# LuisaGroup/LuisaRender

Measured on AMD Instinct MI355X. Metric: Msamples/s (+ fraction of HBM roofline) at fixed SPP, 1/2/4/8 GPU, higher is better.
Workload: dtype f32; 1 GPU; Contemporary Bathroom-class (procedural stand-in, ~600k tris), 1024x1024, 1024spp, depth 16; integrator=MegaPath, sampler=Independent (seed 19980810), spp=1024, parallelism=single GPU, collective=none (single GPU), scheduler=path pool, two contexts per lane (megapool_kernel.h)

## Files before the change

__graft_entry__.py:

```python
import os
import subprocess
import sys

ROOT = os.path.dirname(os.path.abspath(__file__))
if ROOT not in sys.path:
    sys.path.insert(0, ROOT)


def build() -> None:
    jobs = f"-j{min(os.cpu_count() or 4, 16)}"
    subprocess.check_call(["make", "-C", ROOT, jobs, "host", "oracle", "hip", "cli", "ieee", "shallow", "noearly", "nopair", "noride"])
    if os.path.isdir("/root/reference/src"):
        subprocess.check_call(["make", "-C", ROOT, jobs, "ref"])
    import luisarender_amd
    from luisarender_amd import _ffi
    _ffi.host_lib()
    assert os.path.exists(os.path.join(ROOT, "luisarender_amd", "lib", "liblrhip.so"))


def smoke() -> None:
    import numpy as np
    from luisarender_amd import Scene
    from oracle.check import Oracle
    from luisarender_amd.render import MegaPathRenderer
    from luisarender_amd.scenes import cornell_box

    scene = Scene.from_string(cornell_box(resolution=64, spp=8))
    renderer = MegaPathRenderer(0)
    renderer.upload(scene)
    renderer.render(0, 8, counters=True, sync=True)
    gpu = renderer.download(converted=False)
    cpu, counters = Oracle(scene).render(0, 8)
    rel = float(np.abs(gpu[..., :3] - cpu[..., :3]).sum() / np.abs(cpu[..., :3]).sum())
    gc = renderer.counters()
    assert np.array_equal(gpu[..., 3], cpu[..., 3]), "sample counts differ"
    assert abs(gc["closest_rays"] - counters["closest_rays"]) <= 2, (gc, counters)
    assert rel < 1e-4, f"relative L1 vs oracle {rel}"
    print(f"smoke ok: rel L1 vs oracle = {rel:.3e}, {renderer.last_render_ms():.3f} ms")


if __name__ == "__main__":
    build()
    if len(sys.argv) > 1 and sys.argv[1] == "smoke":
        smoke()
```

luisarender_amd/csrc/hip/megapool_kernel.h:

```cpp
#pragma once
#include "dev_wavefront.h"

namespace lrd {

#ifndef LR_MIN_WAVES
#define LR_MIN_WAVES 4
#endif
#ifndef LR_POOL_SHADE_LANES
#define LR_POOL_SHADE_LANES 56
#endif
#ifndef LR_POOL_IDLE_LANES
#define LR_POOL_IDLE_LANES 16
#endif
#ifndef LR_POOL_TURNOVER_LANES
#define LR_POOL_TURNOVER_LANES 12
#endif
#ifndef LR_POOL_PARK_ON_STACK
#define LR_POOL_PARK_ON_STACK 1
#endif
#ifndef LR_POOL_FUSED_FETCH
#define LR_POOL_FUSED_FETCH 1
#endif
#ifndef LR_POOL_FUSED_ALPHA
#define LR_POOL_FUSED_ALPHA 0
#endif
#ifndef LR_POOL_EARLY_FETCH
#define LR_POOL_EARLY_FETCH 1
#endif
#ifndef LR_POOL_LEAF_NODE_PAIR
#define LR_POOL_LEAF_NODE_PAIR 1
#endif
#ifndef LR_POOL_EARLY_TAIL_PRIO
#define LR_POOL_EARLY_TAIL_PRIO 3
#endif
#ifndef LR_POOL_STATE_LEAN
#define LR_POOL_STATE_LEAN 1
#endif
#ifndef LR_POOL_RAY_INIT
#define LR_POOL_RAY_INIT if (!mine)
#endif
#ifndef LR_POOL_SHADOW_RIDE
#define LR_POOL_SHADOW_RIDE 1
#endif
constexpr uint32_t kPoolSlots = 128u;

template<bool GENERIC>
constexpr uint32_t pool_quads() { return GENERIC ? 5u : 4u; }
constexpr uint32_t kPoolRecordQuadsMax = pool_quads<true>() + 1u;
constexpr uint32_t kPoolPending = 1u << 22u;

enum : uint32_t {
    kCtxShadow = 1u, kCtxClosest = 2u,
    kCtxHadShadow = 4u, kCtxHadClosest = 8u,
    kCtxDone = 16u,
    kCtxOccluded = 32u,
    kCtxSide = 64u,
    kCtxOpen = 128u,
};
struct PathCtx {
    f3 so, sd;
    float s_tmax;
    f3 no, nd;
    float n_tmin, n_tmax;
    uint32_t tri;
    float u, v;
    uint32_t flags;
};
LR_D void ctx_start(PathCtx &c, TravState &tr) {
    tr.o = c.no, tr.d = c.nd, tr.t_min = c.n_tmin, tr.t_max = c.n_tmax;
    tr.phase = kPhaseClosest;
    if ((c.flags & kCtxShadow) != 0u) {
        asm volatile("");
        tr.o = c.so, tr.d = c.sd, tr.t_min = 0.f, tr.t_max = c.s_tmax;
        tr.phase = kPhaseShadow;
        c.flags &= ~kCtxShadow;
    } else {
        asm volatile("");
        c.flags &= ~kCtxClosest;
    }
    tr.cur = 0u, tr.sp = 0u;
    tr.hit.tri = kInvalid, tr.hit.u = 0.f, tr.hit.v = 0.f;
    tr.occluded = false;
}

LR_D void swap_words(float &x, float &y) { asm volatile("v_swap_b32 %0, %1" : "+v"(x), "+v"(y)); }
LR_D void swap_words(uint32_t &x, uint32_t &y) { asm volatile("v_swap_b32 %0, %1" : "+v"(x), "+v"(y)); }
LR_D void ctx_swap(PathCtx &a, PathCtx &b) {
    swap_words(a.so.x, b.so.x), swap_words(a.so.y, b.so.y), swap_words(a.so.z, b.so.z), swap_words(a.s_tmax, b.s_tmax);
    swap_words(a.sd.x, b.sd.x), swap_words(a.sd.y, b.sd.y), swap_words(a.sd.z, b.sd.z);
    swap_words(a.no.x, b.no.x), swap_words(a.no.y, b.no.y), swap_words(a.no.z, b.no.z), swap_words(a.n_tmin, b.n_tmin);
    swap_words(a.nd.x, b.nd.x), swap_words(a.nd.y, b.nd.y), swap_words(a.nd.z, b.nd.z), swap_words(a.n_tmax, b.n_tmax);
    swap_words(a.tri, b.tri), swap_words(a.u, b.u), swap_words(a.v, b.v), swap_words(a.flags, b.flags);
}

#ifndef LR_POOL_TURNOVER_MOVES
#define LR_POOL_TURNOVER_MOVES 1
#endif
LR_D void ctx_turnover(PathCtx &a, PathCtx &b) {
    if (LR_POOL_TURNOVER_MOVES == 0) { ctx_swap(a, b); return; }
    a.so = b.so, a.sd = b.sd, a.s_tmax = b.s_tmax, a.n_tmin = b.n_tmin, a.n_tmax = b.n_tmax;
    b.tri = a.tri, b.u = a.u, b.v = a.v;
    swap_words(a.no.x, b.no.x), swap_words(a.no.y, b.no.y), swap_words(a.no.z, b.no.z);
    swap_words(a.nd.x, b.nd.x), swap_words(a.nd.y, b.nd.y), swap_words(a.nd.z, b.nd.z);
    swap_words(a.flags, b.flags);
}

LR_D uint32_t lane_rank(unsigned long long mask) {
    return __builtin_amdgcn_mbcnt_hi(static_cast<uint32_t>(mask >> 32u), __builtin_amdgcn_mbcnt_lo(static_cast<uint32_t>(mask), 0u));
}

constexpr uint32_t kCtxRays = kCtxShadow | kCtxClosest;
LR_D bool ctx_shadeable(uint32_t flags, bool samples_left) {
#ifdef LR_POOL_SINGLE
    if ((flags & kCtxSide) != 0u) { samples_left = false; }
#endif
    return (flags & kCtxDone) != 0u || (samples_left && (flags & kCtxOpen) == 0u);
}
LR_D bool pool_shade_due(uint32_t phase, uint32_t cur_flags, uint32_t oth_flags, bool samples_left) {
    const auto idle = phase == kPhaseIdle;
    const auto s = lr_ballot(ctx_shadeable(oth_flags, samples_left) || (idle && ctx_shadeable(cur_flags, samples_left)));
    if (s == 0ull) { return false; }
    const auto idle_mask = lr_ballot(idle);
    return static_cast<uint32_t>(__popcll(s)) >= static_cast<uint32_t>(LR_POOL_SHADE_LANES) ||
           static_cast<uint32_t>(__popcll(s & idle_mask)) >= static_cast<uint32_t>(LR_POOL_IDLE_LANES) || idle_mask == ~0ull;
}

template<bool COUNT, bool ALPHA>
LR_D bool pool_trace(const DScene &scene, const TraversalStack &stack, TravState &tr, PathCtx &cur, PathCtx &oth, bool samples_left, TraceStats &stats) {
    const auto tl = TravLane::make(scene, stack);
    auto inv = safe_inverse(tr.d);
    auto spb = tl.spb_of(tr.sp);
    if (tr.phase == kPhaseIdle) { tr.cur = kCurIdle; }
    auto for_alpha = false;
    constexpr bool FUSED = LR_POOL_FUSED_FETCH != 0 && (!ALPHA || LR_POOL_FUSED_ALPHA != 0);
    constexpr int EARLY = FUSED ? LR_POOL_EARLY_FETCH : 0;
    constexpr bool PAIR = FUSED && LR_POOL_LEAF_NODE_PAIR != 0;
#ifdef LR_STALL_PROBE
    if (COUNT) { probe_start(stats); }
#endif
    LeafRequest rq;
    [[maybe_unused]] auto asked = tr.cur;
// ... 25 lines not shown
            const auto any_inner = PAIR || lr_any(static_cast<int>(tr.cur) >= 0), deep = lr_any(spb > tl.s_deep);
            trav_consume<COUNT, ALPHA, PAIR>(stack, tl, tr, spb, inv, rq, any_inner, deep, stats);
            trav_requests<COUNT, true, PAIR>(stack, tl, tr, spb, rq, EARLY == 1, stats);
            if (LR_POOL_EARLY_TAIL_PRIO == 0) { prio_tests(); }
            if (COUNT) { asked = tr.cur; }
        } else {
            trav_iteration<COUNT, ALPHA, FUSED, PAIR>(stack, tl, tr, spb, inv, stats);
        }
#ifdef LR_TRACE_PROBE
        const auto probe_t1 = __builtin_readcyclecounter();
        const auto probe_t2 = probe_t1;
#endif
        if (ALPHA && alpha_tests_due(tr.phase, tr.cur)) { for_alpha = true; break; }
        const auto ended = tr.cur == kInvalid;
        const auto n_ended = static_cast<uint32_t>(__popcll(lr_ballot(ended)));
#ifdef LR_TRACE_PROBE
        if (COUNT && (threadIdx.x & 63u) == 0u) {
            stats.nodes_empty += static_cast<uint32_t>(probe_t1 - probe_t0);
            stats.steps_starved += static_cast<uint32_t>(__builtin_readcyclecounter() - probe_t2);
        }
#endif
        if (n_ended == 0u) { continue; }
        if (n_ended < static_cast<uint32_t>(LR_POOL_TURNOVER_LANES) && lr_any(tr.cur < kCurParked)) { continue; }
        if (ended) {
            if (tr.phase == kPhaseShadow) {
                if (tr.occluded) { cur.flags |= kCtxOccluded; }
            } else {
                cur.tri = tr.hit.tri, cur.u = tr.hit.u, cur.v = tr.hit.v;
            }
            tr.phase = kPhaseIdle, tr.cur = kCurIdle;
            if ((cur.flags & kCtxRays) == 0u) {
                cur.flags |= kCtxDone;
                if ((oth.flags & kCtxRays) != 0u) { ctx_turnover(cur, oth); }
            }
            if ((cur.flags & kCtxRays) != 0u) {
                ctx_start(cur, tr);
                inv = safe_inverse(tr.d);
                spb = tl.lds_base;
            }
        }
        if (!lr_any(ended && tr.cur == kCurIdle)) { continue; }
        if (lr_ballot(tr.cur != kCurIdle) == 0ull) { break; }
        if (pool_shade_due(tr.phase, cur.flags, oth.flags, samples_left)) { break; }
    }
    if (EARLY != 0) { trav_fetch_wait(); }
    LR_MARK(kProbeTail, tr.cur);
    prio_shade();
    tr.sp = tl.sp_of(spb);
    return for_alpha;
}

#ifndef LR_PADDED_DRAWS_OUT_OF_LINE
#define LR_PADDED_DRAWS_OUT_OF_LINE 1
#endif
struct PaddedDraws {
    float a, b, c, d;
};
[[maybe_unused]] static __device__ __noinline__ PaddedDraws padded_draws(const DScene *scene, uint32_t sample_index, uint32_t pixel, uint32_t dimension, bool four) {
    PathSampler<true> sampler{};
    uint32_t words[kWfSamplerWordsMax] = {sample_index, 0u, dimension, pixel};
    sampler.restore(*scene, words);
    PaddedDraws r;
    r.a = sampler.next_1d();
    const auto u = sampler.next_2d();
    r.b = u.x, r.c = u.y;
    r.d = four ? sampler.next_1d() : 0.f;
    return r;
}

#ifndef LR_LIGHT_OUT_OF_LINE
#if defined(LR_VARIANT) && ((LR_VARIANT) & 16) && !((LR_VARIANT) & (96 | 256))
#define LR_LIGHT_OUT_OF_LINE 1
#else
#define LR_LIGHT_OUT_OF_LINE 0
#endif
#endif
template<bool ENV>
[[maybe_unused]] static __device__ __noinline__ LightPick sample_one_light_call(const DScene *scene, f3 p, f3 ng, f3 ns, uint32_t offset_bits, float u0, float u1, float u2) {
    SurfacePoint it{};
    it.p = p, it.ng = ng, it.shading.n = ns, it.offset_bits = offset_bits;
    return sample_one_light<ENV>(*scene, it, u0, f2{u1, u2});
}

#define LR_POOL_FILM_ADD(L, PIXEL, OF_ITEM, TILE_PIXEL)                                                                                          \
    do {                                                                                                                                         \
        const auto rgb = (L) * scene.shutter_weight;                                                                                             \
        if (CONT || (OF_ITEM) != item) {                                \
            wf_film_accumulate(scene, args.film, (PIXEL), rgb, scene.film_clamp);                                                                \
        } else if (!(any_nan(rgb) || any_inf(rgb))) {   \
            const auto threshold = scene.film_clamp * fmaxf(1.f, 1.f);                                                                           \
            const auto strength = fmaxf(fmaxf(fmaxf(fabsf(rgb.x), fabsf(rgb.y)), fabsf(rgb.z)), 0.f);                                            \
            const auto c = rgb * (threshold / fmaxf(strength, threshold));                                                                       \
            const auto px_sums = film_tile + (TILE_PIXEL) * 3u;                                                                                  \
            if (c.x != 0.f) { atomicAdd(px_sums + 0, radiance_to_fixed(c.x, scene.wf.accum_scale)); }                                            \
            if (c.y != 0.f) { atomicAdd(px_sums + 1, radiance_to_fixed(c.y, scene.wf.accum_scale)); }                                            \
            if (c.z != 0.f) { atomicAdd(px_sums + 2, radiance_to_fixed(c.z, scene.wf.accum_scale)); }                                            \
        } else {                                                                        \
            atomicAdd(&args.film[(PIXEL)].w, -1.f);                                                                                              \
        }                                                                                                                                        \
    } while (false)

template<uint32_t F>
__global__ __launch_bounds__(kBlockThreads, LR_MIN_WAVES) void megapool_kernel(DScenePtr scene_ptr, RenderArgs args) {
    const DScene &scene = *(const DScene *)scene_ptr;
    constexpr bool COUNT = (F & kFeatCount) != 0u, PCG = (F & kFeatGeneric) != 0u, ENV = (F & kFeatEnv) != 0u,
                   ALPHA = (F & kFeatAlpha) != 0u, DISNEY = (F & kFeatDisney) != 0u, WF = (F & kFeatWf) != 0u, CONT = (F & kFeatCont) != 0u;
    static_assert((F & kFeatPool) != 0u, "a pool variant");
    static_assert(kPoolParkedWords == 5u, "the shading block parks five words on top of a lane's stack (below): lrhip_upload_scene bounds the BVH depth with this constant");
    static_assert((F & (kFeatMix | kFeatLayered | kFeatAux | kFeatVpt | kFeatNest)) == 0u, "the pool scheduler exists for the lean kernels (closures inline)");
    static_assert(!WF || !DISNEY, "a wavefront variant is a lean kernel: the heavy closures live in heavy_kernel.h");
    static_assert(!CONT || WF, "the continuation pass exists in wavefront mode only");
    constexpr uint32_t SAMPLER_WORDS = PathSampler<PCG>::kSavedWords;
#ifdef LR_ONLY_SAMPLER
    constexpr bool PADDED = PCG && (LR_ONLY_SAMPLER) == LR_SAMPLER_PADDED_SOBOL;
#else
    constexpr bool PADDED = false;
#endif
    static_assert(PADDED == ((F & kFeatPadded) != 0u) || (F & kFeatPadded) == 0u, "a kFeatPadded kernel: generic sampler, LR_ONLY_SAMPLER = PaddedSobol");
    constexpr uint32_t QUADS = PADDED ? 4u : pool_quads<PCG>();
    constexpr bool RIDE = LR_POOL_SHADOW_RIDE != 0 && !WF;
    constexpr uint32_t RECORD = QUADS + (RIDE ? 1u : 0u);
    static_assert(RECORD <= kPoolRecordQuadsMax, "ensure_pool sizes the records");
    __shared__ uint32_t s_stack[kStackLds * kBlockThreads];
    __shared__ float4 s_stage[kWavesPerBlock * kStageWave];
#if LR_POOL_PARK_ON_STACK == 0
    __shared__ uint32_t s_park[5u * kBlockThreads];
    static_assert(kStackLds + 5u <= 16u, "the parking area is carved out of the round 1-3 stack: compile such pool variants with LR_STACK_LDS <= 11");
#endif
    __shared__ unsigned long long s_film[CONT ? 1u : kWavesPerBlock * 192u];
#ifdef LR_STALL_PROBE
    __shared__ uint32_t s_probe[kWavesPerBlock * kProbeWords];
    if ((threadIdx.x & 63u) < kProbeWords) { s_probe[(threadIdx.x >> 6u) * kProbeWords + (threadIdx.x & 63u)] = 0u; }
    const auto probe_wave = (F & kFeatCount) != 0u && (blockIdx.x % 9u) == 0u && __builtin_amdgcn_readfirstlane(threadIdx.x >> 6u) == ((blockIdx.x / 9u) & 3u);
#endif
    const auto tid = threadIdx.x;
    const auto lane = tid & 63u;
    const auto gtid = blockIdx.x * kBlockThreads + tid;
    const auto wave_in_block = __builtin_amdgcn_readfirstlane(tid >> 6u);
    TraversalStack stack{s_stack + tid, args.spill + gtid, args.total_threads, s_stage + wave_in_block * kStageWave};
    const auto film_tile = s_film + (CONT ? 0u : wave_in_block * 192u);
    const auto state_of = [&](uint32_t side, uint32_t quad) { return args.pool + static_cast<size_t>(side * RECORD + quad) * args.total_threads + gtid; };
    const auto state_load = [&](uint32_t side, uint32_t quad) { return *state_of(side, quad); };
    const auto state_store = [&](uint32_t side, uint32_t quad, float4 v) { *state_of(side, quad) = v; };
    DCounters local{};
    const auto t_wave = COUNT ? __builtin_readcyclecounter() : 0ull;

    const auto cont_total = CONT ? min(scene.wf.counts[kWfCountCont], scene.wf.capacity) : 0u;
    const auto cont_waves = gridDim.x * kWavesPerBlock;
    const auto item_records = CONT ? min(kWfItemRecords, max(64u, ((cont_total + cont_waves - 1u) / cont_waves + 63u) & ~63u)) : 1u;
    const auto item_count = CONT ? (cont_total + item_records - 1u) / item_records : args.item_count;
    const auto cont_queue = wf_cont_queue(scene);

    auto item = kInvalid;
    auto items_left = true;
    auto q_next = 0u, q_total = 0u;
    auto s_begin = 0u, s_count = 0u, tx = 0u, ty = 0u;
    if (!CONT) { film_tile[lane * 3u] = 0ull, film_tile[lane * 3u + 1u] = 0ull, film_tile[lane * 3u + 2u] = 0ull; }
    TravState tr{};
    tr.phase = kPhaseIdle;
    PathCtx cur{}, oth{};
    cur.flags = 0u, oth.flags = kCtxSide;

    auto flush_tile = [&]() {
        if (CONT || item == kInvalid) { return; }
        __builtin_amdgcn_fence(__ATOMIC_ACQ_REL, "wavefront");
        __builtin_amdgcn_wave_barrier();
        const auto a0 = film_tile[lane * 3u], a1 = film_tile[lane * 3u + 1u], a2 = film_tile[lane * 3u + 2u];
        film_tile[lane * 3u] = 0ull, film_tile[lane * 3u + 1u] = 0ull, film_tile[lane * 3u + 2u] = 0ull;
        const auto wx = tx * 8u + (lane & 7u), wy = ty * 8u + (lane >> 3u);
        if (wx < scene.camera.width && wy < scene.camera.height) {
            const auto index = wy * scene.camera.width + wx;
            const auto acc = scene.wf.accum + static_cast<size_t>(index) * 3u;
            if (a0 != 0ull) { atomicAdd(acc + 0, a0); }
            if (a1 != 0ull) { atomicAdd(acc + 1, a1); }
            if (a2 != 0ull) { atomicAdd(acc + 2, a2); }
            if (s_count != 0u) { atomicAdd(&args.film[index].w, static_cast<float>(s_count)); }
        }
        __builtin_amdgcn_fence(__ATOMIC_ACQ_REL, "wavefront");
        __builtin_amdgcn_wave_barrier();
    };

    auto take_item = [&]() {
        flush_tile();
        item = next_item(CONT ? scene.wf.counts + kWfWorkCont : args.work_counter, item_count, lane);
        q_next = 0u, q_total = 0u, s_count = 0u;
        if (item == kInvalid) {
            items_left = false;
            return;
        }
        if (CONT) {
            q_total = min(item_records, cont_total - item * item_records);
        } else {
            const auto range = item_range(args, item);
            const auto tile = args.tile_begin + range.tile_index * args.tile_stride;
            ty = tile / args.tiles_x, tx = (tile - ty * args.tiles_x + ty) % args.tiles_x;
            s_begin = range.s_begin, s_count = range.s_end > range.s_begin ? range.s_end - range.s_begin : 0u;
            q_total = s_count * 64u;
        }
    };

    for (;;) {
        for (;;) {
            const auto samples_left = items_left || q_next < q_total;
            if (!pool_shade_due(tr.phase, cur.flags, oth.flags, samples_left)) { break; }
            const auto t_shade = COUNT ? __builtin_readcyclecounter() : 0ull;
            if (ALPHA) { tr.pend_t = 0.f, tr.pend_u = 0.f, tr.pend_v = 0.f; }
            if (tr.phase == kPhaseIdle && !ctx_shadeable(oth.flags, samples_left)) { ctx_swap(cur, oth); }
#ifdef LR_POOL_SINGLE
            const auto mine = (oth.flags & kCtxDone) != 0u || ((oth.flags & kCtxOpen) == 0u && (oth.flags & kCtxSide) == 0u);
#else
            const auto mine = (oth.flags & kCtxDone) != 0u || (oth.flags & kCtxOpen) == 0u;
#endif
            {
                const auto stage = stack.stage;
                stage[lane] = make_float4(cur.so.x, cur.so.y, cur.so.z, cur.s_tmax);
                stage[64u + lane] = make_float4(cur.sd.x, cur.sd.y, cur.sd.z, cur.n_tmin);
                stage[128u + lane] = make_float4(cur.no.x, cur.no.y, cur.no.z, cur.n_tmax);
                const auto keep_word = (tr.phase & 7u) | (tr.occluded ? 8u : 0u) | (tr.sp << 5u) | (cur.flags << 12u) | (oth.flags << 20u);
                stage[192u + lane] = make_float4(cur.nd.x, cur.nd.y, cur.nd.z, __uint_as_float(keep_word));
#if LR_POOL_PARK_ON_STACK
                stack.push(tr.sp + 0u, tr.phase != kPhaseIdle ? tr.hit.tri : cur.tri);
                stack.push(tr.sp + 1u, __float_as_uint(tr.phase != kPhaseIdle ? tr.hit.u : cur.u));
                stack.push(tr.sp + 2u, __float_as_uint(tr.phase != kPhaseIdle ? tr.hit.v : cur.v));
                stack.push(tr.sp + 3u, __float_as_uint(tr.t_max));
                stack.push(tr.sp + 4u, tr.cur);
#else
                const auto park = s_park + tid;
                park[0u * kBlockThreads] = tr.phase != kPhaseIdle ? tr.hit.tri : cur.tri;
                park[1u * kBlockThreads] = __float_as_uint(tr.phase != kPhaseIdle ? tr.hit.u : cur.u);
                park[2u * kBlockThreads] = __float_as_uint(tr.phase != kPhaseIdle ? tr.hit.v : cur.v);
                park[3u * kBlockThreads] = __float_as_uint(tr.t_max);
                park[4u * kBlockThreads] = tr.cur;
#endif
                asm volatile("" ::: "memory");
            }
            PathSampler<PCG> sampler{};
            Ray ray{}, shadow{};
            LR_POOL_RAY_INIT {
                shadow.o = oth.so, shadow.d = oth.sd, shadow.t_min = 0.f, shadow.t_max = oth.s_tmax;
                ray.o = oth.no, ray.d = oth.nd, ray.t_min = oth.n_tmin, ray.t_max = oth.n_tmax;
            }
            f3 beta = mk3(0.f), Li = mk3(0.f), nee = mk3(0.f);
            auto pdf_bsdf = 1e16f;
            auto dp = 0u, pixel_index = 0u, path_item = kInvalid;
            const auto side = (oth.flags & kCtxSide) != 0u ? 1u : 0u;
            auto path_open = (oth.flags & kCtxDone) != 0u;
            const auto traced_shadow = path_open && (oth.flags & kCtxHadShadow) != 0u, traced_closest = path_open && (oth.flags & kCtxHadClosest) != 0u;
            const auto occluded = (oth.flags & kCtxOccluded) != 0u;
            const auto ro = oth.no, rd = oth.nd;
            const auto hit_tri = oth.tri;
            const auto hit_u = oth.u, hit_v = oth.v;
            constexpr bool LEAN_STATE = LR_POOL_STATE_LEAN != 0;
            auto word0 = 0u;
            const auto load_ids = [&]() {
                const auto q3 = state_load(side, 3u);
                pixel_index = __float_as_uint(q3.x), path_item = __float_as_uint(q3.y);
            };
            const auto sampler_take = [&](uint32_t stage) {
                if (PADDED) {
                    const auto q3 = state_load(side, 3u);
                    const auto depth = dp & 0xffffu;
                    const auto first_rr = scene.rr_depth == 0u ? 0u : scene.rr_depth - 1u;
                    const auto dimension = (scene.camera.kind == LR_CAMERA_THIN_LENS ? 4u : 2u) + 6u * depth + (depth > first_rr ? depth - first_rr : 0u) + 3u * stage;
                    uint32_t words[kWfSamplerWordsMax] = {__float_as_uint(q3.z), 0u, dimension, __float_as_uint(q3.w)};
                    sampler.restore(scene, words);
                    return;
                }
                const auto q3 = state_load(side, 3u);
                uint32_t words[kWfSamplerWordsMax] = {word0, __float_as_uint(q3.z), __float_as_uint(q3.w), __float_as_uint(state_load(side, QUADS - 1u).x)};
                sampler.restore(scene, words);
            };
            const auto sampler_leave = [&]() {
                if (PADDED) { return; }
                uint32_t words[kWfSamplerWordsMax] = {0u, 0u, 0u, 0u};
                sampler.save(words);
                word0 = words[0];
                state_store(side, 2u, make_float4(Li.x, Li.y, Li.z, __uint_as_float(words[0])));
                const auto q3 = state_load(side, 3u);
                state_store(side, 3u, make_float4(q3.x, q3.y, __uint_as_float(words[1]), __uint_as_float(words[2])));
                state_store(side, QUADS - 1u, make_float4(__uint_as_float(words[3]), 0.f, 0.f, 0.f));
            };
            auto sampler_left = false;
            if (path_open) {
                const auto q0 = state_load(side, 0u), q1 = state_load(side, 1u), q2 = state_load(side, 2u);
                nee = mk3(q0.x, q0.y, q0.z), pdf_bsdf = q0.w;
                beta = mk3(q1.x, q1.y, q1.z);
                const auto packed = __float_as_uint(q1.w);
                dp = packed & (RIDE ? 0x7fffffu : 0x3fffffu);
                Li = mk3(q2.x, q2.y, q2.z);
                word0 = __float_as_uint(q2.w);
                if (!LEAN_STATE) { load_ids(); }
                if (!PCG) {
                    uint32_t words[kWfSamplerWordsMax] = {word0, 0u, 0u, 0u};
                    sampler.restore(scene, words);
                }
            }
            auto want_shadow = false, want_closest = false;
            unsigned long long t_closure_sum = 0ull;
#ifdef LR_STALL_PROBE
            uint32_t t_lobe = 0u, t_eval = 0u, t_sample = 0u, t_hit = 0u, t_light = 0u;
            const auto probe_clock = []() { return static_cast<uint32_t>(__builtin_readcyclecounter()); };
            const auto t_block = probe_clock();
#endif
            auto park_kind = kInvalid;
            if (path_open) {
                if (traced_shadow) {
                    if (!occluded) { Li += nee; }
                }
                if (RIDE && (dp & kPoolPending) != 0u) {
                    const auto ids = state_load(side, QUADS);
                    LR_POOL_FILM_ADD(Li, __float_as_uint(ids.x), __float_as_uint(ids.y), __float_as_uint(ids.z));
                    Li = mk3(0.f), nee = mk3(0.f);
                    dp &= ~kPoolPending;
                }
                if (traced_closest) {
                    if (COUNT) { local.shade_busy++; }
                    const auto wo = -rd;
                    const auto hit_valid = hit_tri != kInvalid;
                    auto u_light_selection = 0.f, u_lobe = 0.f, u_rr = 0.f;
                    f2 u_light_surface{0.f, 0.f}, u_bsdf{0.f, 0.f};
                    const auto rr = (dp & 0xffffu) + 1u >= scene.rr_depth;
                    if (!hit_valid && scene.env_kind != kEnvNone) {
                        f3 L = mk3(scene.env_L[0], scene.env_L[1], scene.env_L[2]);
                        auto pdf = kInvPi * 0.25f;
                        if (ENV && scene.env_kind != kEnvConstant) { env_evaluate(scene, rd, L, pdf); }
                        Li += beta * L * balance(pdf_bsdf, pdf * scene.env_prob);
                    }
                    SurfacePoint it;
                    auto has_surface = false;
#ifdef LR_STALL_PROBE
                    const auto t_h0 = probe_clock();
#endif
                    if (hit_valid) {
                        reconstruct_baked(scene, hit_tri, hit_u, hit_v, it);
                        it.back_facing = dot(wo, it.ng) < 0.0f;
                        if (COUNT) { local.surface_hits++; }
                        if (scene.has_lights && (it.flags & LR_SHAPE_HAS_LIGHT)) {
                            f3 L;
                            float pdf;
                            const auto prim = reinterpret_cast<const uint32_t *>(scene.shade_tris + hit_tri)[29];
                            light_evaluate(scene, it, prim, ro, L, pdf);
                            pdf *= (1.f - scene.env_prob) / static_cast<float>(scene.light_count);
                            Li += beta * L * balance(pdf_bsdf, pdf);
                        }
                        has_surface = (it.flags & LR_SHAPE_HAS_SURFACE) != 0u;
                    }
                    if (WF && has_surface) {
                        const auto heavy_kind = (it.flags >> 10u) & 3u;
                        if (heavy_kind != 0u) { park_kind = heavy_kind - 1u, has_surface = false; }
                    }
                    if (WF) {
                        if (lr_any(park_kind != kInvalid)) {
                            unsigned long long kind_mask[kWfKinds];
#pragma unroll
                            for (auto k = 0u; k < kWfKinds; k++) { kind_mask[k] = lr_ballot(park_kind == k); }
                            static_assert(kWfKinds == 3u, "three closure kinds");
                            const auto my_mask = park_kind == 0u ? kind_mask[0] : (park_kind == 1u ? kind_mask[1] : (park_kind == 2u ? kind_mask[2] : 0ull));
                            auto reserved = 0u;
                            if (my_mask != 0ull && lane == static_cast<uint32_t>(__ffsll(static_cast<long long>(my_mask))) - 1u) {
                                reserved = atomicAdd(scene.wf.counts + kWfCountHeavy + park_kind, static_cast<uint32_t>(__popcll(my_mask)));
                            }
#pragma unroll
                            for (auto k = 0u; k < kWfKinds; k++) {
                                const auto mask = kind_mask[k];
                                if (mask == 0ull) { continue; }
                                const auto leader = __ffsll(static_cast<long long>(mask)) - 1;
                                const auto out = static_cast<uint32_t>(__builtin_amdgcn_readlane(static_cast<int>(reserved), leader)) + lane_rank(mask);
                                if (park_kind == k && out < scene.wf.capacity) {
                                    if (LEAN_STATE) { load_ids(); }
                                    if (PCG) { sampler_take(0u); }
                                    const auto q = wf_heavy_queue<SAMPLER_WORDS>(scene, k);
                                    q.put3(out, 0u, rd);
                                    q.put(out, 3u, hit_tri), q.put(out, 4u, hit_u), q.put(out, 5u, hit_v);
                                    q.put3(out, 6u, beta), q.put3(out, 9u, Li);
                                    q.put(out, 12u, pixel_index), q.put(out, 13u, dp & 0xffffu);
                                    uint32_t words[kWfSamplerWordsMax];
                                    sampler.save(words);
#pragma unroll
                                    for (auto w = 0u; w < SAMPLER_WORDS; w++) { q.put(out, kWfHeavyWords + w, words[w]); }
                                }
                            }
                        }
                    }
#ifdef LR_STALL_PROBE
                    asm volatile("" : "+v"(it.p.x), "+v"(it.ng.x), "+v"(Li.x));
                    const auto t_h1 = probe_clock();
                    t_hit = t_h1 - t_h0;
#endif
                    if (has_surface) {
                        if (COUNT) { local.path_length_sum++, local.nee_samples++; }
                        if constexpr (PADDED && LR_PADDED_DRAWS_OUT_OF_LINE != 0) {
                            sampler_take(0u);
                            const auto r = padded_draws(&scene, sampler.lo, sampler.w3, sampler.w2, false);
                            u_light_selection = r.a, u_light_surface = f2{r.b, r.c};
                        } else {
                            if (PCG) { sampler_take(0u); }
                            u_light_selection = sampler.next_1d();
                            u_light_surface = sampler.next_2d();
                            if (PCG) { sampler_leave(), sampler_left = !PADDED; }
                        }
#if LR_LIGHT_OUT_OF_LINE
                        const auto pick = sample_one_light_call<ENV>(&scene, it.p, it.ng, it.shading.n, it.offset_bits, u_light_selection, u_light_surface.x, u_light_surface.y);
#else
                        const auto pick = sample_one_light<ENV>(scene, it, u_light_selection, u_light_surface);
#endif
                        shadow = pick.shadow;
#ifdef LR_STALL_PROBE
                        asm volatile("" : "+v"(shadow.o.x), "+v"(shadow.d.x));
#endif
                        const auto t_closure = COUNT ? __builtin_readcyclecounter() : 0ull;
#ifdef LR_STALL_PROBE
                        t_light = static_cast<uint32_t>(t_closure) - t_h1;
#endif
                        const LobeTables tables{scene.closures, scene.surfaces, scene.textures, scene.texels};
                        DClosure closure;
                        Frame sh;
                        load_lobe(tables, it.uv, it.ng, wo, (it.tags >> 12u) & 4095u, it.shading, closure, sh);
#ifdef LR_STALL_PROBE
                        asm volatile("" : "+v"(closure.c0[0]), "+v"(closure.s0), "+v"(sh.n.x));
                        const auto t_l1 = probe_clock();
                        t_lobe = t_l1 - static_cast<uint32_t>(t_closure);
#endif
                        if (pick.pdf > 0.0f) {
                            const auto eval = closure_evaluate<DISNEY>(closure, sh, it.ng, wo, shadow.d);
                            const auto w = balance(pick.pdf, eval.pdf) / pick.pdf;
                            nee = w * beta * eval.f * pick.L;
                            want_shadow = nee.x != 0.f || nee.y != 0.f || nee.z != 0.f;
                        }
#ifdef LR_STALL_PROBE
                        asm volatile("" : "+v"(nee.x), "+v"(nee.y), "+v"(nee.z));
                        const auto t_e1 = probe_clock();
                        t_eval = t_e1 - t_l1;
#endif
                        if constexpr (PADDED && LR_PADDED_DRAWS_OUT_OF_LINE != 0) {
                            sampler_take(1u);
                            const auto r = padded_draws(&scene, sampler.lo, sampler.w3, sampler.w2, rr);
                            u_lobe = r.a, u_bsdf = f2{r.b, r.c}, u_rr = r.d;
                        } else {
                            if (PCG) { sampler_take(1u); }
                            u_lobe = sampler.next_1d();
                            u_bsdf = sampler.next_2d();
                            if (PCG) {
                                if (rr) { u_rr = sampler.next_1d(); }
                                sampler_leave();
                            }
                        }
                        const auto bs = closure_sample<DISNEY>(closure, sh, it.ng, wo, u_lobe, u_bsdf);
                        auto eta = 1.f;
                        const auto has_eta = closure_eta(closure, eta);
                        ray.o = robust_origin(it, bs.wi);
                        ray.d = bs.wi;
                        ray.t_min = 0.f, ray.t_max = kFloatMax;
                        pdf_bsdf = bs.pdf;
                        beta *= (bs.pdf > 0.f ? 1.f / bs.pdf : 0.f) * bs.f;
                        auto eta_scale = 1.f;
                        if (has_eta) {
                            if (bs.event == kEventEnter) { eta_scale = sqr(eta); }
                            else if (bs.event == kEventExit) { eta_scale = sqr(1.f / eta); }
                        }
                        if (any_nan(beta)) { beta = mk3(0.f); }
                        auto alive = !(beta.x <= 0.f && beta.y <= 0.f && beta.z <= 0.f);
                        if (!PCG && rr) { u_rr = sampler.next_1d(); }
                        if (alive) {
                            const auto q = fmaxf(max_component(beta) * eta_scale, .05f);
                            if (rr) {
                                if (q < scene.rr_threshold && u_rr >= q) { alive = false; }
                                else { beta *= q < scene.rr_threshold ? 1.0f / q : 1.f; }
                            }
                        }
                        dp++;
                        want_closest = alive && (dp & 0xffffu) < scene.max_depth;
                        if (COUNT) { t_closure_sum += __builtin_readcyclecounter() - t_closure; }
#ifdef LR_STALL_PROBE
                        asm volatile("" : "+v"(beta.x), "+v"(ray.d.x));
                        t_sample = probe_clock() - t_e1;
#endif
                    }
                }
            }
            if (WF) {
                if (park_kind != kInvalid) { path_open = false; }
            }
            if (path_open && !want_shadow && !want_closest) {
                if (LEAN_STATE) { load_ids(); }
                LR_POOL_FILM_ADD(Li, pixel_index, path_item, dp >> 16u);
                path_open = false;
            }
            const auto t_regen = COUNT ? __builtin_readcyclecounter() : 0ull;
            if (COUNT) {
                for (auto off = 32; off > 0; off >>= 1) { t_closure_sum = max(t_closure_sum, static_cast<unsigned long long>(__shfl_xor(static_cast<long long>(t_closure_sum), off))); }
            }
            const auto final_shadow = RIDE && path_open && want_shadow && !want_closest;
            auto need = mine && (!path_open || final_shadow);
            auto got = false;
            auto new_k = 0u, new_item = kInvalid, new_px = 0u, new_py = 0u, new_s = 0u;
            for (;;) {
                const auto mask = lr_ballot(need);
                if (mask == 0ull) { break; }
                if (q_next >= q_total) {
                    if (!items_left) { break; }
                    take_item();
                    if (!items_left) { break; }
                    continue;
                }
                const auto avail = q_total - q_next;
                const auto rank = lane_rank(mask);
                if (need && rank < avail) {
                    const auto k = q_next + rank;
                    const auto px = tx * 8u + (k & 7u), py = ty * 8u + ((k >> 3u) & 7u);
                    if (CONT || (px < scene.camera.width && py < scene.camera.height)) {
                        new_k = k, new_item = item, new_px = px, new_py = py, new_s = s_begin + (k >> 6u);
                        got = true, need = false;
                    }
                }
                q_next += min(static_cast<uint32_t>(__popcll(mask)), avail);
            }
            if (got) {
                sampler_left = false;
                if (CONT) {
                    const auto rec = new_item * item_records + new_k;
                    const auto &q = cont_queue;
                    ray.o = q.get3(rec, 0u), ray.d = q.get3(rec, 3u);
                    ray.t_min = 0.f, ray.t_max = kFloatMax;
                    shadow.o = q.get3(rec, 6u), shadow.d = q.get3(rec, 9u);
                    shadow.t_min = 0.f, shadow.t_max = q.getf(rec, 12u);
                    nee = q.get3(rec, 13u), beta = q.get3(rec, 16u), Li = q.get3(rec, 19u);
                    pdf_bsdf = q.getf(rec, 22u);
                    pixel_index = q.get(rec, 23u);
                    const auto packed = q.get(rec, 24u);
                    dp = packed & 0xffffu;
                    want_shadow = (packed & (1u << 16u)) != 0u, want_closest = (packed & (1u << 17u)) != 0u;
                    uint32_t words[kWfSamplerWordsMax];
#pragma unroll
                    for (auto w = 0u; w < SAMPLER_WORDS; w++) { words[w] = q.get(rec, kWfContWords + w); }
                    sampler.restore(scene, words);
                    path_open = true;
                } else {
                    if (final_shadow) {
                        if (LEAN_STATE) { load_ids(); }
                        state_store(side, QUADS, make_float4(__uint_as_float(pixel_index), __uint_as_float(path_item), __uint_as_float(dp >> 16u), 0.f));
                    }
                    pixel_index = new_py * scene.camera.width + new_px;
                    path_item = new_item;
                    sampler.start(scene, new_px, new_py, new_s);
                    const auto u_filter = sampler.next_pixel_2d();
                    const auto u_lens = scene.camera.kind == LR_CAMERA_THIN_LENS ? sampler.next_2d() : f2{.5f, .5f};
                    float weight;
                    camera_ray(scene, scene.filter, new_px, new_py, u_filter, u_lens, ray, weight);
                    beta = mk3(weight);
                    if (!final_shadow) { Li = mk3(0.f), nee = mk3(0.f); }
                    pdf_bsdf = 1e16f;
                    dp = ((new_k & 63u) << 16u) | (final_shadow ? kPoolPending : 0u);
                    path_open = true, want_shadow = final_shadow, want_closest = true;
                    if (COUNT) { local.paths++; }
                }
            }
            const auto t_launch = COUNT ? __builtin_readcyclecounter() : 0ull;
            const auto go = path_open && (want_shadow || want_closest);
            if (go) {
                state_store(side, 0u, make_float4(nee.x, nee.y, nee.z, pdf_bsdf));
                state_store(side, 1u, make_float4(beta.x, beta.y, beta.z, __uint_as_float(dp)));
                if (!PCG || !sampler_left) {
                    uint32_t words[kWfSamplerWordsMax] = {word0, 0u, 0u, 0u};
                    if (!PCG || got) { sampler.save(words); }
                    state_store(side, 2u, make_float4(Li.x, Li.y, Li.z, __uint_as_float(words[0])));
                    if (got && PADDED) {
                        state_store(side, 3u, make_float4(__uint_as_float(pixel_index), __uint_as_float(path_item), __uint_as_float(words[0]), __uint_as_float(words[3])));
                    } else if (got) {
                        state_store(side, 3u, make_float4(__uint_as_float(pixel_index), __uint_as_float(path_item), __uint_as_float(words[1]), __uint_as_float(words[2])));
                        if (PCG) { state_store(side, QUADS - 1u, make_float4(__uint_as_float(words[3]), 0.f, 0.f, 0.f)); }
                    } else if (!LEAN_STATE && !PCG) {
                        state_store(side, 3u, make_float4(__uint_as_float(pixel_index), __uint_as_float(path_item), 0.f, 0.f));
                    }
                }
                if (COUNT) { local.closest_rays += want_closest ? 1u : 0u, local.shadow_rays += want_shadow ? 1u : 0u; }
            }
            {
                const auto stage = stack.stage;
                asm volatile("" ::: "memory");
                const auto p0 = stage[lane], p1 = stage[64u + lane], p2 = stage[128u + lane], p3 = stage[192u + lane];
                cur.so = mk3(p0.x, p0.y, p0.z), cur.s_tmax = p0.w;
                cur.sd = mk3(p1.x, p1.y, p1.z), cur.n_tmin = p1.w;
                cur.no = mk3(p2.x, p2.y, p2.z), cur.n_tmax = p2.w;
                cur.nd = mk3(p3.x, p3.y, p3.z);
                const auto keep_word = __float_as_uint(p3.w);
                tr.phase = keep_word & 7u, tr.occluded = (keep_word & 8u) != 0u;
                tr.sp = (keep_word >> 5u) & 127u;
#if LR_POOL_PARK_ON_STACK
                const auto keep_tri = stack.pop(tr.sp + 0u);
                const auto keep_u = __uint_as_float(stack.pop(tr.sp + 1u)), keep_v = __uint_as_float(stack.pop(tr.sp + 2u));
                tr.t_max = __uint_as_float(stack.pop(tr.sp + 3u)), tr.cur = stack.pop(tr.sp + 4u);
#else
                const auto park = s_park + tid;
                const auto keep_tri = park[0u * kBlockThreads];
                const auto keep_u = __uint_as_float(park[1u * kBlockThreads]), keep_v = __uint_as_float(park[2u * kBlockThreads]);
                tr.t_max = __uint_as_float(park[3u * kBlockThreads]), tr.cur = park[4u * kBlockThreads];
#endif
                cur.flags = (keep_word >> 12u) & 0xffu, cur.tri = keep_tri, cur.u = keep_u, cur.v = keep_v;
                tr.hit.tri = keep_tri, tr.hit.u = keep_u, tr.hit.v = keep_v;
                __builtin_amdgcn_fence(__ATOMIC_ACQ_REL, "wavefront");
                oth.so = shadow.o, oth.sd = shadow.d, oth.s_tmax = shadow.t_max;
                oth.no = ray.o, oth.nd = ray.d, oth.n_tmin = ray.t_min, oth.n_tmax = ray.t_max;
                oth.tri = kInvalid, oth.u = 0.f, oth.v = 0.f;
                const auto shaded_flags = (side != 0u ? kCtxSide : 0u) |
                                          (go ? kCtxOpen | (want_shadow ? kCtxShadow | kCtxHadShadow : 0u) | (want_closest ? kCtxClosest | kCtxHadClosest : 0u) : 0u);
                oth.flags = mine ? shaded_flags : (keep_word >> 20u) & 0xffu;
                if ((tr.phase & 3u) == kPhaseShadow) { tr.o = cur.so, tr.d = cur.sd, tr.t_min = 0.f; }
                else { tr.o = cur.no, tr.d = cur.nd, tr.t_min = cur.n_tmin; }
            }
            if (tr.phase == kPhaseIdle && (oth.flags & kCtxRays) != 0u) {
                ctx_swap(cur, oth);
                ctx_start(cur, tr);
            }
#ifdef LR_STALL_PROBE
            if (COUNT) {
                const auto wave_max = [](uint32_t v) {
                    for (auto off = 32; off > 0; off >>= 1) { v = max(v, static_cast<uint32_t>(__shfl_xor(static_cast<int>(v), off))); }
                    return v;
                };
                const auto m_hit = wave_max(t_hit), m_light = wave_max(t_light), m_lobe = wave_max(t_lobe), m_eval = wave_max(t_eval), m_sample = wave_max(t_sample);
                if (probe_wave && lane == 0u) {
                    atomicAdd(&args.counters->probe[14], 1ull);
                    atomicAdd(&args.counters->probe[15], static_cast<unsigned long long>(probe_clock() - t_block));
                    atomicAdd(&args.counters->probe[8], static_cast<unsigned long long>(m_hit + m_light));
                    atomicAdd(&args.counters->probe[9], static_cast<unsigned long long>(m_lobe));
                    atomicAdd(&args.counters->probe[10], static_cast<unsigned long long>(m_eval));
                    atomicAdd(&args.counters->probe[11], static_cast<unsigned long long>(m_sample));
                }
            }
#endif
            if (COUNT) {
                if (lane == 0u) {
                    const auto t_end = __builtin_readcyclecounter();
                    local.shade_cycles += t_end - t_shade;
                    local.shade_closure_cycles += t_closure_sum, local.shade_regen_cycles += t_launch - t_regen;
                    local.shade_light_cycles += (t_regen - t_shade) - t_closure_sum;
                }
                local.shade_calls++;
            }
        }
        if (!lr_any(tr.phase != kPhaseIdle)) { break; }
        TraceStats ts{};
#ifdef LR_STALL_PROBE
        ts.probe_lds = probe_wave ? static_cast<uint32_t>(reinterpret_cast<uintptr_t>((TraversalStack::lds_u32 *)(s_probe + wave_in_block * kProbeWords))) : 0u;
#endif
        const auto t_trace = COUNT ? __builtin_readcyclecounter() : 0ull;
        for (;;) {
            const auto for_alpha = pool_trace<COUNT, ALPHA>(scene, stack, tr, cur, oth, items_left || q_next < q_total, ts);
            if (!ALPHA) { break; }
            if (lr_any((tr.phase & kPhasePendingAlpha) != 0u)) { resolve_pending_alpha(scene, stack, tr); }
            if (!for_alpha) { break; }
        }
#ifdef LR_STALL_PROBE
        if (COUNT && ts.probe_lds != 0u && lane == 0u) {
            const auto words = s_probe + wave_in_block * kProbeWords;
#pragma unroll
            for (auto i = 0u; i < kProbeSlots; i++) { atomicAdd(&args.counters->probe[i], static_cast<unsigned long long>(words[i])), words[i] = 0u; }
            atomicAdd(&args.counters->probe[12], static_cast<unsigned long long>(ts.steps));
            atomicAdd(&args.counters->probe[13], static_cast<unsigned long long>(__builtin_readcyclecounter() - t_trace));
        }
#endif
        if (COUNT) {
            if (lane == 0u) { local.trace_cycles += __builtin_readcyclecounter() - t_trace; }
            local.nodes_visited += ts.nodes, local.tris_tested += ts.tris, local.nodes_empty += ts.nodes_empty;
            local.trace_steps += ts.steps, local.trace_steps_busy += ts.steps_busy, local.trace_steps_starved += ts.steps_starved;
#ifndef LR_STALL_PROBE
            if (ts.early_fetch_broken != 0u) { atomicAdd(&args.counters->probe[kProbeEarlyFetchBroken], static_cast<unsigned long long>(ts.early_fetch_broken)); }
#endif
        }
    }
    flush_tile();

    if (COUNT) {
        if (lane == 0u) { local.wave_cycles = __builtin_readcyclecounter() - t_wave; }
        auto reduce = [&](unsigned long long v, unsigned long long *dst) {
            for (auto off = 32; off > 0; off >>= 1) { v += __shfl_down(v, off); }
            if (lane == 0u) { atomicAdd(dst, v); }
        };
        reduce(local.paths, &args.counters->paths);
        reduce(local.closest_rays, &args.counters->closest_rays);
        reduce(local.shadow_rays, &args.counters->shadow_rays);
        reduce(local.nodes_visited, &args.counters->nodes_visited);
        reduce(local.tris_tested, &args.counters->tris_tested);
        reduce(local.surface_hits, &args.counters->surface_hits);
        reduce(local.nee_samples, &args.counters->nee_samples);
        reduce(local.path_length_sum, &args.counters->path_length_sum);
        reduce(local.trace_steps, &args.counters->trace_steps);
        reduce(local.trace_steps_busy, &args.counters->trace_steps_busy);
        reduce(local.shade_calls, &args.counters->shade_calls);
        reduce(local.shade_busy, &args.counters->shade_busy);
        reduce(local.trace_steps_starved, &args.counters->trace_steps_starved);
        reduce(local.shade_cycles, &args.counters->shade_cycles);
        reduce(local.trace_cycles, &args.counters->trace_cycles);
        reduce(local.wave_cycles, &args.counters->wave_cycles);
        reduce(local.nodes_empty, &args.counters->nodes_empty);
        reduce(local.shade_light_cycles, &args.counters->shade_light_cycles);
        reduce(local.shade_closure_cycles, &args.counters->shade_closure_cycles);
        reduce(local.shade_regen_cycles, &args.counters->shade_regen_cycles);
    }
}

#undef LR_POOL_FILM_ADD

// ... 2 lines not shown
```

Baseline: 1287 Msamples/s.

## Track path item staleness with flag bits instead of reloading per-path ids

```diff
diff --git a/__graft_entry__.py b/__graft_entry__.py
--- a/__graft_entry__.py
+++ b/__graft_entry__.py
@@ -9,7 +9,7 @@
 
 def build() -> None:
     jobs = f"-j{min(os.cpu_count() or 4, 16)}"
-    subprocess.check_call(["make", "-C", ROOT, jobs, "host", "oracle", "hip", "cli", "ieee", "shallow", "noearly", "nopair", "noride"])
+    subprocess.check_call(["make", "-C", ROOT, jobs, "host", "oracle", "hip", "cli", "ieee", "shallow", "noearly", "nopair", "noride", "nolazy"])
     if os.path.isdir("/root/reference/src"):
         subprocess.check_call(["make", "-C", ROOT, jobs, "ref"])
     import luisarender_amd
diff --git a/luisarender_amd/csrc/hip/megapool_kernel.h b/luisarender_amd/csrc/hip/megapool_kernel.h
--- a/luisarender_amd/csrc/hip/megapool_kernel.h
+++ b/luisarender_amd/csrc/hip/megapool_kernel.h
@@ -41,13 +41,24 @@
 #endif
 #ifndef LR_POOL_SHADOW_RIDE
 #define LR_POOL_SHADOW_RIDE 1
+#endif
+#ifndef LR_POOL_IDS_LAZY
+#define LR_POOL_IDS_LAZY 1
 #endif
 constexpr uint32_t kPoolSlots = 128u;
 
 template<bool GENERIC>
 constexpr uint32_t pool_quads() { return GENERIC ? 5u : 4u; }
 constexpr uint32_t kPoolRecordQuadsMax = pool_quads<true>() + 1u;
+constexpr uint32_t kPoolDepthMask = 0xffffu, kPoolTileShift = 16u, kPoolTileMask = 63u;
 constexpr uint32_t kPoolPending = 1u << 22u;
+constexpr uint32_t kPoolIdsExtra = 1u << 23u;
+constexpr uint32_t kPoolOldTileShift = 24u, kPoolOldStale = 1u << 30u;
+constexpr uint32_t kPoolOldBits = (kPoolTileMask << kPoolOldTileShift) | kPoolOldStale;
+static_assert(kPoolDepthMask == (1u << kPoolTileShift) - 1u, "the depth keeps its 16 bits (lrhip_render sends deeper paths to the one-path kernels)");
+static_assert(((kPoolTileMask << kPoolTileShift) & (kPoolPending | kPoolIdsExtra | kPoolOldBits)) == 0u && (kPoolPending & (kPoolIdsExtra | kPoolOldBits)) == 0u &&
+                  (kPoolIdsExtra & kPoolOldBits) == 0u && (kPoolOldBits >> 31u) == 0u,
+              "the fields of the depth word do not overlap");
 
 enum : uint32_t {
     kCtxShadow = 1u, kCtxClosest = 2u,
@@ -56,7 +67,15 @@
     kCtxOccluded = 32u,
     kCtxSide = 64u,
     kCtxOpen = 128u,
+    kCtxStale = 256u,
 };
+constexpr uint32_t kKeepSpShift = 5u, kKeepSpMask = 127u, kKeepCurShift = 12u;
+constexpr uint32_t keep_flag_bits(bool stale) { return stale ? 9u : 8u; }
+constexpr uint32_t keep_flags_mask(bool stale) { return (1u << keep_flag_bits(stale)) - 1u; }
+constexpr uint32_t keep_oth_shift(bool stale) { return kKeepCurShift + keep_flag_bits(stale); }
+static_assert(kCtxStale <= keep_flags_mask(true) && kCtxStale > keep_flags_mask(false) && kCtxOpen <= keep_flags_mask(false), "every flag of a context fits its field of the keep word");
+static_assert(kKeepSpShift + 7u <= kKeepCurShift && (kKeepSpMask >> 7u) == 0u && keep_oth_shift(true) + keep_flag_bits(true) <= 32u && keep_oth_shift(false) + keep_flag_bits(false) <= 32u,
+              "the fields of the keep word do not overlap");
 struct PathCtx {
     f3 so, sd;
     float s_tmax;
@@ -248,10 +267,10 @@
     return sample_one_light<ENV>(*scene, it, u0, f2{u1, u2});
 }
 
-#define LR_POOL_FILM_ADD(L, PIXEL, OF_ITEM, TILE_PIXEL)                                                                                          \
+#define LR_POOL_FILM_ADD(L, PIXEL, STRAGGLER, TILE_PIXEL)                                                                                        \
     do {                                                                                                                                         \
         const auto rgb = (L) * scene.shutter_weight;                                                                                             \
-        if (CONT || (OF_ITEM) != item) {                                \
+        if (CONT || (STRAGGLER)) {                                      \
             wf_film_accumulate(scene, args.film, (PIXEL), rgb, scene.film_clamp);                                                                \
         } else if (!(any_nan(rgb) || any_inf(rgb))) {   \
             const auto threshold = scene.film_clamp * fmaxf(1.f, 1.f);                                                                           \
@@ -287,6 +306,8 @@
     constexpr bool RIDE = LR_POOL_SHADOW_RIDE != 0 && !WF;
     constexpr uint32_t RECORD = QUADS + (RIDE ? 1u : 0u);
     static_assert(RECORD <= kPoolRecordQuadsMax, "ensure_pool sizes the records");
+    constexpr bool LAZY = LR_POOL_IDS_LAZY != 0 && !WF && !PCG;
+    constexpr uint32_t KEEP_FLAGS = keep_flags_mask(LAZY), KEEP_OTH = keep_oth_shift(LAZY);
     __shared__ uint32_t s_stack[kStackLds * kBlockThreads];
     __shared__ float4 s_stage[kWavesPerBlock * kStageWave];
 #if LR_POOL_PARK_ON_STACK == 0
@@ -321,6 +342,7 @@
     auto items_left = true;
     auto q_next = 0u, q_total = 0u;
     auto s_begin = 0u, s_count = 0u, tx = 0u, ty = 0u;
+    [[maybe_unused]] auto item_changed = false;
     if (!CONT) { film_tile[lane * 3u] = 0ull, film_tile[lane * 3u + 1u] = 0ull, film_tile[lane * 3u + 2u] = 0ull; }
     TravState tr{};
     tr.phase = kPhaseIdle;
@@ -348,6 +370,7 @@
 
     auto take_item = [&]() {
         flush_tile();
+        if constexpr (LAZY) { item_changed = true; }
         item = next_item(CONT ? scene.wf.counts + kWfWorkCont : args.work_counter, item_count, lane);
         q_next = 0u, q_total = 0u, s_count = 0u;
         if (item == kInvalid) {
@@ -382,7 +405,7 @@
                 stage[lane] = make_float4(cur.so.x, cur.so.y, cur.so.z, cur.s_tmax);
                 stage[64u + lane] = make_float4(cur.sd.x, cur.sd.y, cur.sd.z, cur.n_tmin);
                 stage[128u + lane] = make_float4(cur.no.x, cur.no.y, cur.no.z, cur.n_tmax);
-                const auto keep_word = (tr.phase & 7u) | (tr.occluded ? 8u : 0u) | (tr.sp << 5u) | (cur.flags << 12u) | (oth.flags << 20u);
+                const auto keep_word = (tr.phase & 7u) | (tr.occluded ? 8u : 0u) | (tr.sp << kKeepSpShift) | (cur.flags << kKeepCurShift) | (oth.flags << KEEP_OTH);
                 stage[192u + lane] = make_float4(cur.nd.x, cur.nd.y, cur.nd.z, __uint_as_float(keep_word));
 #if LR_POOL_PARK_ON_STACK
                 stack.push(tr.sp + 0u, tr.phase != kPhaseIdle ? tr.hit.tri : cur.tri);
@@ -410,6 +433,8 @@
             auto pdf_bsdf = 1e16f;
             auto dp = 0u, pixel_index = 0u, path_item = kInvalid;
             const auto side = (oth.flags & kCtxSide) != 0u ? 1u : 0u;
+            [[maybe_unused]] const auto stale_in = [&]() { return ((__float_as_uint(stack.stage[192u + lane].w) >> KEEP_OTH) & kCtxStale) != 0u; };
+            if constexpr (LAZY) { item_changed = false; }
             auto path_open = (oth.flags & kCtxDone) != 0u;
             const auto traced_shadow = path_open && (oth.flags & kCtxHadShadow) != 0u, traced_closest = path_open && (oth.flags & kCtxHadClosest) != 0u;
             const auto occluded = (oth.flags & kCtxOccluded) != 0u;
@@ -418,10 +443,33 @@
             const auto hit_u = oth.u, hit_v = oth.v;
             constexpr bool LEAN_STATE = LR_POOL_STATE_LEAN != 0;
             auto word0 = 0u;
+#ifdef LR_STALL_PROBE_ENTRY
+            uint32_t t_entry = 0u, t_hitrec = 0u, t_ids = 0u;
+            const auto entry_clock = []() { return static_cast<uint32_t>(__builtin_readcyclecounter()); };
+#endif
             const auto load_ids = [&]() {
+#ifdef LR_STALL_PROBE_ENTRY
+                const auto t_i0 = entry_clock();
+#endif
                 const auto q3 = state_load(side, 3u);
                 pixel_index = __float_as_uint(q3.x), path_item = __float_as_uint(q3.y);
+#ifdef LR_STALL_PROBE_ENTRY
+                asm volatile("" : "+v"(pixel_index), "+v"(path_item));
+                t_ids += entry_clock() - t_i0;
+#endif
             };
+            const auto ids_quad = [](uint32_t word, bool other = false) { return LAZY && RIDE && ((word & kPoolIdsExtra) != 0u) != other ? QUADS : 3u; };
+#ifdef LR_STALL_PROBE_ENTRY
+            [[maybe_unused]] const auto lazy_pixel = [&](uint32_t word, bool other) {
+                const auto t_i0 = entry_clock();
+                auto pixel = __float_as_uint(state_load(side, ids_quad(word, other)).x);
+                asm volatile("" : "+v"(pixel));
+                t_ids += entry_clock() - t_i0;
+                return pixel;
+            };
+#else
+            [[maybe_unused]] const auto lazy_pixel = [&](uint32_t word, bool other) { return __float_as_uint(state_load(side, ids_quad(word, other)).x); };
+#endif
             const auto sampler_take = [&](uint32_t stage) {
                 if (PADDED) {
                     const auto q3 = state_load(side, 3u);
@@ -447,12 +495,16 @@
                 state_store(side, QUADS - 1u, make_float4(__uint_as_float(words[3]), 0.f, 0.f, 0.f));
             };
             auto sampler_left = false;
+            static_assert(!LAZY || LEAN_STATE, "LR_POOL_IDS_LAZY reads the ids where they are needed: it has no form that reads them at every vertex");
+#ifdef LR_STALL_PROBE_ENTRY
+            const auto t_e0 = entry_clock();
+#endif
             if (path_open) {
                 const auto q0 = state_load(side, 0u), q1 = state_load(side, 1u), q2 = state_load(side, 2u);
                 nee = mk3(q0.x, q0.y, q0.z), pdf_bsdf = q0.w;
                 beta = mk3(q1.x, q1.y, q1.z);
                 const auto packed = __float_as_uint(q1.w);
-                dp = packed & (RIDE ? 0x7fffffu : 0x3fffffu);
+                dp = packed & (RIDE ? (LAZY ? 0x7fffffffu : 0x7fffffu) : 0x3fffffu);
                 Li = mk3(q2.x, q2.y, q2.z);
                 word0 = __float_as_uint(q2.w);
                 if (!LEAN_STATE) { load_ids(); }
@@ -460,6 +512,10 @@
                     uint32_t words[kWfSamplerWordsMax] = {word0, 0u, 0u, 0u};
                     sampler.restore(scene, words);
                 }
+#ifdef LR_STALL_PROBE_ENTRY
+                asm volatile("" : "+v"(nee.x), "+v"(beta.x), "+v"(dp), "+v"(Li.x));
+                t_entry = entry_clock() - t_e0;
+#endif
             }
             auto want_shadow = false, want_closest = false;
             unsigned long long t_closure_sum = 0ull;
@@ -474,8 +530,20 @@
                     if (!occluded) { Li += nee; }
                 }
                 if (RIDE && (dp & kPoolPending) != 0u) {
-                    const auto ids = state_load(side, QUADS);
-                    LR_POOL_FILM_ADD(Li, __float_as_uint(ids.x), __float_as_uint(ids.y), __float_as_uint(ids.z));
+                    if constexpr (LAZY) {
+                        LR_POOL_FILM_ADD(Li, lazy_pixel(dp, true), stale_in() || (dp & kPoolOldStale) != 0u, (dp >> kPoolOldTileShift) & kPoolTileMask);
+                        dp &= ~kPoolOldBits;
+                    } else {
+#ifdef LR_STALL_PROBE_ENTRY
+                        const auto t_i0 = entry_clock();
+                        auto ids = state_load(side, QUADS);
+                        asm volatile("" : "+v"(ids.x), "+v"(ids.y), "+v"(ids.z));
+                        t_ids += entry_clock() - t_i0;
+#else
+                        const auto ids = state_load(side, QUADS);
+#endif
+                        LR_POOL_FILM_ADD(Li, __float_as_uint(ids.x), __float_as_uint(ids.y) != item, __float_as_uint(ids.z));
+                    }
                     Li = mk3(0.f), nee = mk3(0.f);
                     dp &= ~kPoolPending;
                 }
@@ -498,7 +566,14 @@
                     const auto t_h0 = probe_clock();
 #endif
                     if (hit_valid) {
+#ifdef LR_STALL_PROBE_ENTRY
+                        const auto t_r0 = entry_clock();
+#endif
                         reconstruct_baked(scene, hit_tri, hit_u, hit_v, it);
+#ifdef LR_STALL_PROBE_ENTRY
+                        asm volatile("" : "+v"(it.p.x), "+v"(it.ng.x), "+v"(it.uv.x), "+v"(it.shading.n.x), "+v"(it.flags), "+v"(it.tags), "+v"(it.offset_bits), "+v"(it.tri_offset));
+                        t_hitrec = entry_clock() - t_r0;
+#endif
                         it.back_facing = dot(wo, it.ng) < 0.0f;
                         if (COUNT) { local.surface_hits++; }
                         if (scene.has_lights && (it.flags & LR_SHAPE_HAS_LIGHT)) {
@@ -648,8 +723,12 @@
                 if (park_kind != kInvalid) { path_open = false; }
             }
             if (path_open && !want_shadow && !want_closest) {
-                if (LEAN_STATE) { load_ids(); }
-                LR_POOL_FILM_ADD(Li, pixel_index, path_item, dp >> 16u);
+                if constexpr (LAZY) {
+                    LR_POOL_FILM_ADD(Li, lazy_pixel(dp, false), stale_in(), (dp >> kPoolTileShift) & kPoolTileMask);
+                } else {
+                    if (LEAN_STATE) { load_ids(); }
+                    LR_POOL_FILM_ADD(Li, pixel_index, path_item != item, dp >> 16u);
+                }
                 path_open = false;
             }
             const auto t_regen = COUNT ? __builtin_readcyclecounter() : 0ull;
@@ -680,6 +759,15 @@
                     }
                 }
                 q_next += min(static_cast<uint32_t>(__popcll(mask)), avail);
+            }
+            if constexpr (LAZY) {
+                if (item_changed) {
+                    auto &parked = stack.stage[192u + lane].w;
+                    auto word = __float_as_uint(parked);
+                    if (((word >> kKeepCurShift) & kCtxOpen) != 0u) { word |= kCtxStale << kKeepCurShift; }
+                    if (((word >> KEEP_OTH) & kCtxOpen) != 0u) { word |= kCtxStale << KEEP_OTH; }
+                    parked = __uint_as_float(word);
+                }
             }
             if (got) {
                 sampler_left = false;
@@ -702,7 +790,7 @@
                     sampler.restore(scene, words);
                     path_open = true;
                 } else {
-                    if (final_shadow) {
+                    if (!LAZY && final_shadow) {
                         if (LEAN_STATE) { load_ids(); }
                         state_store(side, QUADS, make_float4(__uint_as_float(pixel_index), __uint_as_float(path_item), __uint_as_float(dp >> 16u), 0.f));
                     }
@@ -716,7 +804,13 @@
                     beta = mk3(weight);
                     if (!final_shadow) { Li = mk3(0.f), nee = mk3(0.f); }
                     pdf_bsdf = 1e16f;
-                    dp = ((new_k & 63u) << 16u) | (final_shadow ? kPoolPending : 0u);
+                    if constexpr (LAZY) {
+                        const auto old_stale = stale_in();
+                        const auto old_bits = kPoolPending | (~dp & kPoolIdsExtra) | (((dp >> kPoolTileShift) & kPoolTileMask) << kPoolOldTileShift) | (old_stale ? kPoolOldStale : 0u);
+                        dp = ((new_k & 63u) << kPoolTileShift) | (final_shadow ? old_bits : 0u);
+                    } else {
+                        dp = ((new_k & 63u) << 16u) | (final_shadow ? kPoolPending : 0u);
+                    }
                     path_open = true, want_shadow = final_shadow, want_closest = true;
                     if (COUNT) { local.paths++; }
                 }
@@ -733,7 +827,8 @@
                     if (got && PADDED) {
                         state_store(side, 3u, make_float4(__uint_as_float(pixel_index), __uint_as_float(path_item), __uint_as_float(words[0]), __uint_as_float(words[3])));
                     } else if (got) {
-                        state_store(side, 3u, make_float4(__uint_as_float(pixel_index), __uint_as_float(path_item), __uint_as_float(words[1]), __uint_as_float(words[2])));
+                        if constexpr (LAZY) { state_store(side, ids_quad(dp), make_float4(__uint_as_float(pixel_index), __uint_as_float(path_item), __uint_as_float(words[1]), __uint_as_float(words[2]))); }
+                        else { state_store(side, 3u, make_float4(__uint_as_float(pixel_index), __uint_as_float(path_item), __uint_as_float(words[1]), __uint_as_float(words[2]))); }
                         if (PCG) { state_store(side, QUADS - 1u, make_float4(__uint_as_float(words[3]), 0.f, 0.f, 0.f)); }
                     } else if (!LEAN_STATE && !PCG) {
                         state_store(side, 3u, make_float4(__uint_as_float(pixel_index), __uint_as_float(path_item), 0.f, 0.f));
@@ -751,7 +846,7 @@
                 cur.nd = mk3(p3.x, p3.y, p3.z);
                 const auto keep_word = __float_as_uint(p3.w);
                 tr.phase = keep_word & 7u, tr.occluded = (keep_word & 8u) != 0u;
-                tr.sp = (keep_word >> 5u) & 127u;
+                tr.sp = (keep_word >> kKeepSpShift) & kKeepSpMask;
 #if LR_POOL_PARK_ON_STACK
                 const auto keep_tri = stack.pop(tr.sp + 0u);
                 const auto keep_u = __uint_as_float(stack.pop(tr.sp + 1u)), keep_v = __uint_as_float(stack.pop(tr.sp + 2u));
@@ -762,15 +857,16 @@
                 const auto keep_u = __uint_as_float(park[1u * kBlockThreads]), keep_v = __uint_as_float(park[2u * kBlockThreads]);
                 tr.t_max = __uint_as_float(park[3u * kBlockThreads]), tr.cur = park[4u * kBlockThreads];
 #endif
-                cur.flags = (keep_word >> 12u) & 0xffu, cur.tri = keep_tri, cur.u = keep_u, cur.v = keep_v;
+                cur.flags = (keep_word >> kKeepCurShift) & KEEP_FLAGS, cur.tri = keep_tri, cur.u = keep_u, cur.v = keep_v;
                 tr.hit.tri = keep_tri, tr.hit.u = keep_u, tr.hit.v = keep_v;
                 __builtin_amdgcn_fence(__ATOMIC_ACQ_REL, "wavefront");
                 oth.so = shadow.o, oth.sd = shadow.d, oth.s_tmax = shadow.t_max;
                 oth.no = ray.o, oth.nd = ray.d, oth.n_tmin = ray.t_min, oth.n_tmax = ray.t_max;
                 oth.tri = kInvalid, oth.u = 0.f, oth.v = 0.f;
                 const auto shaded_flags = (side != 0u ? kCtxSide : 0u) |
-                                          (go ? kCtxOpen | (want_shadow ? kCtxShadow | kCtxHadShadow : 0u) | (want_closest ? kCtxClosest | kCtxHadClosest : 0u) : 0u);
-                oth.flags = mine ? shaded_flags : (keep_word >> 20u) & 0xffu;
+                                          (go ? kCtxOpen | (want_shadow ? kCtxShadow | kCtxHadShadow : 0u) | (want_closest ? kCtxClosest | kCtxHadClosest : 0u) : 0u) |
+                                          (LAZY && go && (got ? new_item != item : ((keep_word >> KEEP_OTH) & kCtxStale) != 0u) ? kCtxStale : 0u);
+                oth.flags = mine ? shaded_flags : (keep_word >> KEEP_OTH) & KEEP_FLAGS;
                 if ((tr.phase & 3u) == kPhaseShadow) { tr.o = cur.so, tr.d = cur.sd, tr.t_min = 0.f; }
                 else { tr.o = cur.no, tr.d = cur.nd, tr.t_min = cur.n_tmin; }
             }
@@ -784,7 +880,12 @@
                     for (auto off = 32; off > 0; off >>= 1) { v = max(v, static_cast<uint32_t>(__shfl_xor(static_cast<int>(v), off))); }
                     return v;
                 };
+#ifdef LR_STALL_PROBE_ENTRY
+                const auto m_hit = wave_max(t_entry), m_light = 0u, m_lobe = wave_max(t_hitrec), m_eval = wave_max(t_ids), m_sample = 0u;
+                (void)t_hit, (void)t_light, (void)t_lobe, (void)t_eval, (void)t_sample;
+#else
                 const auto m_hit = wave_max(t_hit), m_light = wave_max(t_light), m_lobe = wave_max(t_lobe), m_eval = wave_max(t_eval), m_sample = wave_max(t_sample);
+#endif
                 if (probe_wave && lane == 0u) {
                     atomicAdd(&args.counters->probe[14], 1ull);
                     atomicAdd(&args.counters->probe[15], static_cast<unsigned long long>(probe_clock() - t_block));
```

Measured after the change: 1299 Msamples/s (median of 6 runs). About the same (+0.9%).
